# uber/petastorm

Measured on AMD Instinct MI355X. Metric: samples/sec/node (make_batch_reader->PyTorch DataLoader), imagenet config, higher is better.
Workload: dtype fp32; 1 GPU; model=ImageNetSchema(224x224x3 jpeg CompressedImageCodec + int32 label), global_batch=256, parallelism=dp1, prime_batches=0

## Files before the change

petastorm_amd/ops/csrc/ext.cpp:

```cpp
#include <torch/extension.h>

namespace psa {

void snappy_decompress_batch(torch::Tensor comp, torch::Tensor comp_start,
                             torch::Tensor comp_end, torch::Tensor out,
                             torch::Tensor out_offsets,
                             torch::Tensor out_len, torch::Tensor status);
void lz4_decompress_batch(torch::Tensor comp, torch::Tensor blk_start,
                          torch::Tensor blk_end, torch::Tensor out,
                          torch::Tensor out_offsets, torch::Tensor out_len,
                          torch::Tensor status);

void zstd_decompress_host(torch::Tensor src, torch::Tensor src_off,
                          torch::Tensor src_len, torch::Tensor dst,
                          torch::Tensor dst_off, torch::Tensor dst_len,
                          torch::Tensor status);

int64_t zstd_work_bytes();
void zstd_decompress_batch(torch::Tensor src, torch::Tensor src_off,
                           torch::Tensor src_len, torch::Tensor dst,
                           torch::Tensor dst_off, torch::Tensor dst_len,
                           torch::Tensor work, torch::Tensor status);

void rle_hybrid_decode_batch(torch::Tensor data, torch::Tensor start,
                             torch::Tensor end, torch::Tensor bit_width,
                             torch::Tensor n_values, torch::Tensor out_off,
                             torch::Tensor out, torch::Tensor status);
void byte_array_offsets_batch(torch::Tensor data, torch::Tensor start,
                              torch::Tensor end, torch::Tensor n_values,
                              torch::Tensor out_off, torch::Tensor val_off,
                              torch::Tensor val_len, torch::Tensor status);
void varlen_gather(torch::Tensor src, torch::Tensor src_off,
                   torch::Tensor lengths, torch::Tensor dst,
                   torch::Tensor dst_off);
void plain_fixed_decode_batch(torch::Tensor page_buf,
                              torch::Tensor payload_start,
                              torch::Tensor payload_end,
                              torch::Tensor n_values, torch::Tensor row0,
                              int64_t def_mode, int64_t esize,
                              int64_t fill_pattern, torch::Tensor def_buf,
                              torch::Tensor def_start, torch::Tensor def_len,
                              torch::Tensor out,
                              torch::Tensor valid_out, torch::Tensor status);
void npy_payload_offsets(torch::Tensor data, torch::Tensor val_off,
                         torch::Tensor val_len, torch::Tensor pay_off,
                         torch::Tensor pay_len, torch::Tensor status);
void nhwc_to_nchw_normalize(torch::Tensor in, torch::Tensor out,
                            torch::Tensor mean, torch::Tensor inv_std,
                            double scale);
py::dict jpeg_parse_batch(torch::Tensor buf, torch::Tensor val_off,
                          torch::Tensor val_len);
py::dict parquet_walk_pages(torch::Tensor buf, torch::Tensor chunk_off,
                            torch::Tensor chunk_len);
void inflate_batch(torch::Tensor src, torch::Tensor seg_off,
                   torch::Tensor seg_len, torch::Tensor seg_first,
                   torch::Tensor seg_count, torch::Tensor dst,
                   torch::Tensor dst_off, torch::Tensor dst_cap,
                   torch::Tensor produced, int64_t mode,
                   torch::Tensor status);
void png_unfilter_batch(torch::Tensor raw, torch::Tensor raw_off,
                        torch::Tensor out, torch::Tensor out_off,
                        torch::Tensor height, torch::Tensor row_bytes,
                        torch::Tensor bpp, torch::Tensor status);
void bswap16(torch::Tensor data);
py::dict png_parse_batch(torch::Tensor buf, torch::Tensor val_off,
                         torch::Tensor val_len);
py::dict byte_array_host_offsets(torch::Tensor buf, torch::Tensor val_start,
                                 torch::Tensor counts);
void jpeg_decode_batch(torch::Tensor data, py::dict meta, torch::Tensor coef,
                       torch::Tensor samples, torch::Tensor out,
                       torch::Tensor out_off, torch::Tensor status);
void delta_binary_packed_batch(torch::Tensor page_buf, torch::Tensor start,
                               torch::Tensor end, torch::Tensor n_values,
                               torch::Tensor out_off, torch::Tensor out,
                               int64_t esize, torch::Tensor status);
void delta_length_byte_array_batch(torch::Tensor page_buf,
                                   torch::Tensor start, torch::Tensor end,
                                   torch::Tensor n_values,
                                   torch::Tensor out_idx,
                                   torch::Tensor val_off,
                                   torch::Tensor val_len,
                                   torch::Tensor status);
void delta_byte_array_lengths_batch(torch::Tensor page_buf,
                                    torch::Tensor start, torch::Tensor end,
                                    torch::Tensor n_values,
                                    torch::Tensor out_idx,
                                    torch::Tensor pre, torch::Tensor sfx,
                                    torch::Tensor suf_data_pos,
                                    torch::Tensor status);
void delta_byte_array_reconstruct_batch(
    torch::Tensor page_buf, torch::Tensor n_values, torch::Tensor out_idx,
    torch::Tensor pre, torch::Tensor sfx, torch::Tensor suf_data_pos,
    torch::Tensor val_off, torch::Tensor out, torch::Tensor status);
void byte_stream_split_batch(torch::Tensor page_buf, torch::Tensor start,
                             torch::Tensor n_values, torch::Tensor out_off,
                             torch::Tensor out, int64_t esize);
void bool_unpack_batch(torch::Tensor page_buf, torch::Tensor start,
                       torch::Tensor n_values, torch::Tensor out_off,
                       torch::Tensor out);
void jpeg_decode_fused_batch(torch::Tensor data, py::dict meta,
                             torch::Tensor coef, torch::Tensor samples,
                             torch::Tensor out, torch::Tensor out_off,
                             torch::Tensor mean, torch::Tensor inv_std,
                             double scale, torch::Tensor status);

}

PYBIND11_MODULE(TORCH_EXTENSION_NAME, m) {
  m.doc() = "petastorm_amd MI355X (gfx950) decode kernels";
  m.def("snappy_decompress_batch", &psa::snappy_decompress_batch,
        "Batched snappy page decompression (wave-per-page)");
  m.def("lz4_decompress_batch", &psa::lz4_decompress_batch,
        "batch LZ4 block decompression, one wave per block");
  m.def("zstd_decompress_host", &psa::zstd_decompress_host,
        "batch ZSTD frame decompression on host threads (from-scratch "
        "RFC 8878 decoder, GIL released)");
  m.def("zstd_work_bytes", &psa::zstd_work_bytes,
        "per-frame device workspace size for zstd_decompress_batch");
  m.def("zstd_decompress_batch", &psa::zstd_decompress_batch,
        "batch ZSTD frame decompression on device (thread per frame)");
  m.def("rle_hybrid_decode_batch", &psa::rle_hybrid_decode_batch,
        "Parquet RLE/bit-packed hybrid decode (levels & dict indices)");
  m.def("byte_array_offsets_batch", &psa::byte_array_offsets_batch,
        "PLAIN byte-array page -> per-value (offset, length)");
  m.def("varlen_gather", &psa::varlen_gather,
        "Unaligned variable-length byte gather (funnel-shift copy)");
  m.def("plain_fixed_decode_batch", &psa::plain_fixed_decode_batch,
        "Fused PLAIN data-page decode: def levels + prefix scan + scatter");
  m.def("npy_payload_offsets", &psa::npy_payload_offsets,
        ".npy container -> payload (offset, length)");
  m.def("nhwc_to_nchw_normalize", &psa::nhwc_to_nchw_normalize,
        "Fused uint8 NHWC -> float NCHW normalize (LDS-tiled)");
  m.def("parquet_walk_pages", &psa::parquet_walk_pages,
        "Walk Parquet page headers (thrift compact) in a raw column chunk");
  m.def("inflate_batch", &psa::inflate_batch,
        "Batched DEFLATE inflate (zlib/raw), thread-per-stream");
  m.def("png_unfilter_batch", &psa::png_unfilter_batch,
        "PNG scanline unfilter (wave-per-image, bpp-lane chains)");
  m.def("bswap16", &psa::bswap16, "byte-swap 16-bit samples in place");
  m.def("png_parse_batch", &psa::png_parse_batch,
        "Host-side PNG container parse");
  m.def("byte_array_host_offsets", &psa::byte_array_host_offsets,
        "Host-side PLAIN byte-array offset scan");
  m.def("jpeg_parse_batch", &psa::jpeg_parse_batch,
        "Host-side JPEG header/segment parse");
  m.def("jpeg_decode_batch", &psa::jpeg_decode_batch,
        "GPU baseline JPEG decode (huffman/idct/color kernels)");
  m.def("delta_binary_packed_batch", &psa::delta_binary_packed_batch,
        "DELTA_BINARY_PACKED page decode (wave-per-page, shfl prefix scan)");
  m.def("delta_length_byte_array_batch",
        &psa::delta_length_byte_array_batch,
        "DELTA_LENGTH_BYTE_ARRAY page -> per-value (offset, length)");
  m.def("delta_byte_array_lengths_batch",
        &psa::delta_byte_array_lengths_batch,
        "DELTA_BYTE_ARRAY pass 1: prefix/suffix lengths");
  m.def("delta_byte_array_reconstruct_batch",
        &psa::delta_byte_array_reconstruct_batch,
        "DELTA_BYTE_ARRAY pass 2: materialize front-coded values");
  m.def("byte_stream_split_batch", &psa::byte_stream_split_batch,
        "BYTE_STREAM_SPLIT de-interleave");
  m.def("bool_unpack_batch", &psa::bool_unpack_batch,
        "PLAIN boolean bit-unpack");
  m.def("jpeg_decode_fused_batch", &psa::jpeg_decode_fused_batch,
        "JPEG decode with fused YCbCr->RGB + normalize + NCHW fp32 "
        "epilogue (skips the NHWC uint8 intermediate)");
}
```

petastorm_amd/ops/csrc/jpeg.hip:

```cpp
#include <hip/hip_runtime.h>
#include <torch/extension.h>
#include <c10/hip/HIPStream.h>
#include "common.h"

namespace psa {

__constant__ int ZIGZAG_NAT[64] = {
    0,  1,  8,  16, 9,  2,  3,  10, 17, 24, 32, 25, 18, 11, 4,  5,
    12, 19, 26, 33, 40, 48, 41, 34, 27, 20, 13, 6,  7,  14, 21, 28,
    35, 42, 49, 56, 57, 50, 43, 36, 29, 22, 15, 23, 30, 37, 44, 51,
    58, 59, 52, 45, 38, 31, 39, 46, 53, 60, 61, 54, 47, 55, 62, 63};

__constant__ float IDCT_B[8][8] = {
    {0.35355339f, 0.35355339f, 0.35355339f, 0.35355339f,
     0.35355339f, 0.35355339f, 0.35355339f, 0.35355339f},
    {0.49039264f, 0.41573481f, 0.27778512f, 0.09754516f,
     -0.09754516f, -0.27778512f, -0.41573481f, -0.49039264f},
    {0.46193977f, 0.19134172f, -0.19134172f, -0.46193977f,
     -0.46193977f, -0.19134172f, 0.19134172f, 0.46193977f},
    {0.41573481f, -0.09754516f, -0.49039264f, -0.27778512f,
     0.27778512f, 0.49039264f, 0.09754516f, -0.41573481f},
    {0.35355339f, -0.35355339f, -0.35355339f, 0.35355339f,
     0.35355339f, -0.35355339f, -0.35355339f, 0.35355339f},
    {0.27778512f, -0.49039264f, 0.09754516f, 0.41573481f,
     -0.41573481f, -0.09754516f, 0.49039264f, -0.27778512f},
    {0.19134172f, -0.46193977f, 0.46193977f, -0.19134172f,
     -0.19134172f, 0.46193977f, -0.46193977f, 0.19134172f},
    {0.09754516f, -0.27778512f, 0.41573481f, -0.49039264f,
     0.49039264f, -0.41573481f, 0.27778512f, -0.09754516f}};

struct JpegTables {
  const int32_t* lut;
  const int32_t* maxcode;
  const int32_t* mincode;
  const int32_t* valptr;
  const uint8_t* huffval;
  const float* qtabs;
};

struct JpegGeom {
  const int32_t* comp_h;
  const int32_t* comp_v;
  const int32_t* comp_q;
  const int32_t* comp_dc;
  const int32_t* comp_ac;
  const int64_t* samp_off;
  const int32_t* samp_stride;
  const int32_t* mcus_x;
  const int32_t* mcus_y;
  const int32_t* ncomp;
  const int32_t* width;
  const int32_t* height;
  const int64_t* img_block0;
  const int32_t* bpm;
  const int32_t* kmap;
};


struct BitReader {
  const uint8_t* p;
  int64_t pos, end;
  uint64_t buf;
  int cnt;
  uint32_t sw0, sw1;
  int64_t spos;
  int scount;

  __device__ void init(const uint8_t* data, int64_t lo, int64_t hi) {
    p = data; pos = lo; end = hi; buf = 0; cnt = 0; scount = 0; spos = 0;
  }
  __device__ __forceinline__ void fill() {
    while (cnt <= 32) {
      if (pos + 4 <= end) {
        uint32_t w;
        if (scount > 0 && spos == pos) {
          w = sw0;
          sw0 = sw1;
          spos += 4;
          --scount;
        } else {
          scount = 0;
          w = (uint32_t)p[pos] | ((uint32_t)p[pos + 1] << 8) |
              ((uint32_t)p[pos + 2] << 16) | ((uint32_t)p[pos + 3] << 24);
          if (pos + 12 <= end) {
            sw0 = (uint32_t)p[pos + 4] | ((uint32_t)p[pos + 5] << 8) |
// ... 11 lines not shown
            spos = pos + 4;
            scount = 1;
          }
        }
        uint32_t inv = ~w;
        if (!((inv - 0x01010101u) & ~inv & 0x80808080u)) {
          uint32_t be = __builtin_bswap32(w);
          buf |= (uint64_t)be << (32 - cnt);
          cnt += 32;
          pos += 4;
          continue;
        }
      }
      uint8_t b = 0;
      if (pos < end) {
        b = p[pos];
        if (b == 0xFF) {
          if (pos + 1 < end && p[pos + 1] == 0x00) {
            pos += 2;
          } else {
            pos = end;
            b = 0;
          }
        } else {
          pos += 1;
        }
      } else {
        buf |= 0;
        cnt += 8;
        continue;
      }
      buf |= (uint64_t)b << (56 - cnt);
      cnt += 8;
    }
  }
  __device__ __forceinline__ uint32_t peek(int n) {
    return (uint32_t)(buf >> (64 - n));
  }
  __device__ __forceinline__ void consume(int n) {
    buf <<= n;
    cnt -= n;
  }
};

__device__ __forceinline__ int huff_decode(BitReader& br,
                                           const JpegTables& t, int tid) {
  br.fill();
  uint32_t look = br.peek(8);
  int32_t hit = t.lut[tid * 256 + look];
  if (hit >= 0) {
    br.consume(hit >> 16);
    return hit & 0xFF;
  }
  for (int l = 9; l <= 16; ++l) {
    int32_t code = (int32_t)br.peek(l);
    int32_t mc = t.maxcode[tid * 18 + l];
    if (mc >= 0 && code <= mc) {
      br.consume(l);
      int idx = t.valptr[tid * 18 + l] + code - t.mincode[tid * 18 + l];
      return t.huffval[tid * 256 + idx];
    }
  }
  return -1;
}

__device__ __forceinline__ int receive_extend(BitReader& br, int s) {
  br.fill();
  int v = (int)br.peek(s);
  br.consume(s);
  if (v < (1 << (s - 1))) v += (-1 << s) + 1;
  return v;
}

template <bool NT>
__device__ __forceinline__ int decode_block(BitReader& br,
                                            const JpegTables& tabs,
                                            const float* __restrict__ q,
                                            int dc_t, int ac_t,
                                            float* __restrict__ out,
                                            int& pred) {
  int t = huff_decode(br, tabs, dc_t);
  if (t < 0 || t > 15) return 10;
  int diff = t ? receive_extend(br, t) : 0;
  pred += diff;
  if (NT) __builtin_nontemporal_store((float)pred * q[0], out);
  else out[0] = (float)pred * q[0];
  int kk = 1;
  while (kk < 64) {
    int rs = huff_decode(br, tabs, ac_t);
    if (rs < 0) return 11;
    int r = rs >> 4, sz = rs & 15;
    if (sz == 0) {
      if (r != 15) break;
      kk += 16;
    } else {
      kk += r;
      if (kk > 63) return 12;
      int v = receive_extend(br, sz);
      if (NT) __builtin_nontemporal_store((float)v * q[kk],
                                          out + ZIGZAG_NAT[kk]);
      else out[ZIGZAG_NAT[kk]] = (float)v * q[kk];
      ++kk;
    }
  }
  return 0;
}

template <bool NT>
__global__ void jpeg_huffman_kernel(
    const uint8_t* __restrict__ data, JpegTables tabs, JpegGeom g,
    const int32_t* __restrict__ seg_img, const int64_t* __restrict__ seg_pos,
    const int64_t* __restrict__ seg_end, const int32_t* __restrict__ seg_mcu0,
    const int32_t* __restrict__ seg_nmcu, float* __restrict__ coef,
    int32_t* __restrict__ status, int n_segs) {
  int s = blockIdx.x * blockDim.x + threadIdx.x;
  if (s >= n_segs) return;
// ... 42 lines not shown

__global__ void jpeg_idct_kernel(const float* __restrict__ coef,
                                 JpegGeom g, uint8_t* __restrict__ samples,
                                 int n_imgs, int64_t block_total) {
  int64_t b = (int64_t)blockIdx.x * blockDim.x + threadIdx.x;
  if (b >= block_total) return;
  int lo = 0, hi = n_imgs - 1;
  while (lo < hi) {
    int mid = (lo + hi + 1) >> 1;
    if (g.img_block0[mid] <= b) lo = mid; else hi = mid - 1;
  }
  const int img = lo;
  const int bpm = g.bpm[img];
  const int64_t r = b - g.img_block0[img];
  const int m = (int)(r / bpm);
  const int k = (int)(r % bpm);
  const int km = g.kmap[img * 8 + k];
  const int c = km >> 8, v = (km >> 4) & 15, h = km & 15;
  const int mx = m % g.mcus_x[img];
  const int my = m / g.mcus_x[img];
  const int stride = g.samp_stride[img * 3 + c];
  uint8_t* dst = samples + g.samp_off[img * 3 + c] +
                 ((int64_t)(my * g.comp_v[img * 3 + c] + v) * 8) * stride +
                 (int64_t)(mx * g.comp_h[img * 3 + c] + h) * 8;

  const float* C = coef + b * 64;
  float tmp[64];
#pragma unroll
  for (int vv = 0; vv < 8; ++vv) {
#pragma unroll
    for (int x = 0; x < 8; ++x) {
      float acc = 0.f;
#pragma unroll
      for (int u = 0; u < 8; ++u) acc += C[vv * 8 + u] * IDCT_B[u][x];
      tmp[vv * 8 + x] = acc;
    }
  }
#pragma unroll
  for (int y = 0; y < 8; ++y) {
    uint8_t row[8];
#pragma unroll
    for (int x = 0; x < 8; ++x) {
      float acc = 0.f;
#pragma unroll
      for (int vv = 0; vv < 8; ++vv) acc += tmp[vv * 8 + x] * IDCT_B[vv][y];
      int pix = __float2int_rn(acc) + 128;
      row[x] = (uint8_t)min(255, max(0, pix));
    }
    *(uint64_t*)(dst + (int64_t)y * stride) = *(const uint64_t*)row;
  }
}


__device__ __forceinline__ int fancy_sample(const uint8_t* plane, int stride,
                                            int cw, int ch, int x, int y,
                                            int sx, int sy) {
  if (sx == 1 && sy == 1) return plane[(int64_t)y * stride + x] << 4;
  int i = x, j = y, dx = 0, dy = 0;
  if (sx == 2) { i = x >> 1; dx = x & 1; }
  if (sy == 2) { j = y >> 1; dy = y & 1; }
  int i2 = min(max(dx ? i + 1 : i - 1, 0), cw - 1);
  int j2 = min(max(dy ? j + 1 : j - 1, 0), ch - 1);
  if (sx == 2 && sy == 2) {
    int t0 = 3 * plane[(int64_t)j * stride + i] +
             plane[(int64_t)j2 * stride + i];
    int t1 = 3 * plane[(int64_t)j * stride + i2] +
             plane[(int64_t)j2 * stride + i2];
    return (3 * t0 + t1 + (dx ? 7 : 8));
  }
  if (sx == 2) {
    int a = plane[(int64_t)j * stride + i], bq = plane[(int64_t)j * stride + i2];
    return (3 * a + bq + (dx ? 2 : 1)) << 2;
  }
  int a = plane[(int64_t)j * stride + i], bq = plane[(int64_t)j2 * stride + i];
  return (3 * a + bq + (dy ? 2 : 1)) << 2;
}

__global__ void jpeg_color_kernel(const uint8_t* __restrict__ samples,
                                  JpegGeom g,
                                  uint8_t* __restrict__ out,
                                  const int64_t* __restrict__ out_off,
                                  int n_imgs) {
  const int img = blockIdx.y;
  const int W = g.width[img], H = g.height[img];
  const int64_t npix = (int64_t)W * H;
  const int nc = g.ncomp[img];
  const uint8_t* yplane = samples + g.samp_off[img * 3 + 0];
  const int ystride = g.samp_stride[img * 3 + 0];
  uint8_t* dst = out + out_off[img];

  const int hmax = g.comp_h[img * 3 + 0];
  const int vmax = g.comp_v[img * 3 + 0];

  const int Wq = (W + 3) >> 2;
  const int64_t nquads = (int64_t)Wq * H;
  const uint8_t* cbp = samples + g.samp_off[img * 3 + 1];
  const uint8_t* crp = samples + g.samp_off[img * 3 + 2];
  const int cstride = g.samp_stride[img * 3 + 1];
  const int cw = (W + hmax - 1) / hmax;
  const int chh = (H + vmax - 1) / vmax;

  for (int64_t q = (int64_t)blockIdx.x * blockDim.x + threadIdx.x;
       q < nquads; q += (int64_t)gridDim.x * blockDim.x) {
    const int y = (int)(q / Wq);
    const int x0 = (int)(q % Wq) << 2;
    const int cnt = min(4, W - x0);
    const int64_t pix0 = (int64_t)y * W + x0;
    const uint8_t* yrow = yplane + (int64_t)y * ystride + x0;

    if (nc == 1) {
      if (cnt == 4 && (((uintptr_t)(dst + pix0) & 3) == 0) &&
          (((uintptr_t)yrow & 3) == 0))
        *(uint32_t*)(dst + pix0) = *(const uint32_t*)yrow;
      else
        for (int k = 0; k < cnt; ++k) dst[pix0 + k] = yrow[k];
      continue;
    }

    uint8_t rgb[12];
    uint32_t y4 = (cnt == 4) ? load_u32_unaligned(yrow) : 0;
    for (int k = 0; k < cnt; ++k) {
      const int x = x0 + k;
      const float fy = (cnt == 4) ? (float)((y4 >> (8 * k)) & 0xff)
                                  : (float)yrow[k];
      float cb = fancy_sample(cbp, cstride, cw, chh, x, y, hmax, vmax)
                     * (1.f / 16.f) - 128.f;
      float cr = fancy_sample(crp, cstride, cw, chh, x, y, hmax, vmax)
                     * (1.f / 16.f) - 128.f;
      int rv = __float2int_rn(fy + 1.40200f * cr);
      int gv = __float2int_rn(fy - 0.34414f * cb - 0.71414f * cr);
      int bv = __float2int_rn(fy + 1.77200f * cb);
      rgb[k * 3 + 0] = (uint8_t)min(255, max(0, rv));
      rgb[k * 3 + 1] = (uint8_t)min(255, max(0, gv));
      rgb[k * 3 + 2] = (uint8_t)min(255, max(0, bv));
    }
    uint8_t* d = dst + pix0 * 3;
    if (cnt == 4 && (((uintptr_t)d & 3) == 0)) {
      ((uint32_t*)d)[0] = *(const uint32_t*)(rgb + 0);
      ((uint32_t*)d)[1] = *(const uint32_t*)(rgb + 4);
      ((uint32_t*)d)[2] = *(const uint32_t*)(rgb + 8);
    } else {
      for (int k = 0; k < cnt * 3; ++k) d[k] = rgb[k];
    }
  }
}

__global__ void jpeg_color_norm_kernel(
    const uint8_t* __restrict__ samples, JpegGeom g,
    float* __restrict__ out, const int64_t* __restrict__ out_off,
    const float* __restrict__ mean, const float* __restrict__ inv_std,
    float scale, int n_imgs) {
  const int img = blockIdx.y;
  const int W = g.width[img], H = g.height[img];
  const int64_t plane = (int64_t)W * H;
  const int nc = g.ncomp[img];
  const uint8_t* yplane = samples + g.samp_off[img * 3 + 0];
  const int ystride = g.samp_stride[img * 3 + 0];
  float* dst = out + out_off[img];

  const int hmax = g.comp_h[img * 3 + 0];
  const int vmax = g.comp_v[img * 3 + 0];
  const int Wq = (W + 3) >> 2;
  const int64_t nquads = (int64_t)Wq * H;
  const uint8_t* cbp = samples + g.samp_off[img * 3 + 1];
  const uint8_t* crp = samples + g.samp_off[img * 3 + 2];
  const int cstride = g.samp_stride[img * 3 + 1];
  const int cw = (W + hmax - 1) / hmax;
  const int chh = (H + vmax - 1) / vmax;
  const float m0 = mean[0], m1 = mean[1], m2 = mean[2];
  const float s0 = inv_std[0], s1 = inv_std[1], s2 = inv_std[2];

  for (int64_t q = (int64_t)blockIdx.x * blockDim.x + threadIdx.x;
       q < nquads; q += (int64_t)gridDim.x * blockDim.x) {
    const int y = (int)(q / Wq);
    const int x0 = (int)(q % Wq) << 2;
    const int cnt = min(4, W - x0);
    const int64_t pix0 = (int64_t)y * W + x0;
    const uint8_t* yrow = yplane + (int64_t)y * ystride + x0;

    float rpix[4], gpix[4], bpix[4];
    uint32_t y4 = (cnt == 4) ? load_u32_unaligned(yrow) : 0;
    for (int k = 0; k < cnt; ++k) {
      const int x = x0 + k;
      const float fy = (cnt == 4) ? (float)((y4 >> (8 * k)) & 0xff)
                                  : (float)yrow[k];
      int rv, gv, bv;
      if (nc == 1) {
        rv = gv = bv = (int)fy;
      } else {
        float cb = fancy_sample(cbp, cstride, cw, chh, x, y, hmax, vmax)
                       * (1.f / 16.f) - 128.f;
        float cr = fancy_sample(crp, cstride, cw, chh, x, y, hmax, vmax)
                       * (1.f / 16.f) - 128.f;
        rv = __float2int_rn(fy + 1.40200f * cr);
        gv = __float2int_rn(fy - 0.34414f * cb - 0.71414f * cr);
        bv = __float2int_rn(fy + 1.77200f * cb);
      }
      rpix[k] = ((float)min(255, max(0, rv)) * scale - m0) * s0;
      gpix[k] = ((float)min(255, max(0, gv)) * scale - m1) * s1;
      bpix[k] = ((float)min(255, max(0, bv)) * scale - m2) * s2;
    }
    float* dr = dst + pix0;
    float* dg = dst + plane + pix0;
    float* db = dst + 2 * plane + pix0;
    if (cnt == 4 && ((pix0 & 3) == 0)) {
      *(float4*)dr = make_float4(rpix[0], rpix[1], rpix[2], rpix[3]);
      *(float4*)dg = make_float4(gpix[0], gpix[1], gpix[2], gpix[3]);
      *(float4*)db = make_float4(bpix[0], bpix[1], bpix[2], bpix[3]);
    } else {
      for (int k = 0; k < cnt; ++k) {
        dr[k] = rpix[k];
        dg[k] = gpix[k];
        db[k] = bpix[k];
      }
    }
  }
}


static JpegTables make_tables(const py::dict& d) {
  JpegTables t;
  t.lut = d["lut"].cast<torch::Tensor>().data_ptr<int32_t>();
  t.maxcode = d["maxcode"].cast<torch::Tensor>().data_ptr<int32_t>();
  t.mincode = d["mincode"].cast<torch::Tensor>().data_ptr<int32_t>();
  t.valptr = d["valptr"].cast<torch::Tensor>().data_ptr<int32_t>();
  t.huffval = d["huffval"].cast<torch::Tensor>().data_ptr<uint8_t>();
  t.qtabs = d["qtabs"].cast<torch::Tensor>().data_ptr<float>();
  return t;
}

static JpegGeom make_geom(const py::dict& d) {
  JpegGeom g;
  g.comp_h = d["comp_h"].cast<torch::Tensor>().data_ptr<int32_t>();
  g.comp_v = d["comp_v"].cast<torch::Tensor>().data_ptr<int32_t>();
  g.comp_q = d["comp_q"].cast<torch::Tensor>().data_ptr<int32_t>();
  g.comp_dc = d["comp_dc"].cast<torch::Tensor>().data_ptr<int32_t>();
  g.comp_ac = d["comp_ac"].cast<torch::Tensor>().data_ptr<int32_t>();
  g.samp_off = d["samp_off"].cast<torch::Tensor>().data_ptr<int64_t>();
  g.samp_stride = d["samp_stride"].cast<torch::Tensor>().data_ptr<int32_t>();
  g.mcus_x = d["mcus_x"].cast<torch::Tensor>().data_ptr<int32_t>();
  g.mcus_y = d["mcus_y"].cast<torch::Tensor>().data_ptr<int32_t>();
  g.ncomp = d["ncomp"].cast<torch::Tensor>().data_ptr<int32_t>();
  g.width = d["width"].cast<torch::Tensor>().data_ptr<int32_t>();
  g.height = d["height"].cast<torch::Tensor>().data_ptr<int32_t>();
  g.img_block0 = d["img_block0"].cast<torch::Tensor>().data_ptr<int64_t>();
  g.bpm = d["bpm"].cast<torch::Tensor>().data_ptr<int32_t>();
  g.kmap = d["kmap"].cast<torch::Tensor>().data_ptr<int32_t>();
  return g;
}

void jpeg_decode_batch(torch::Tensor data, py::dict meta, torch::Tensor coef,
                       torch::Tensor samples, torch::Tensor out,
                       torch::Tensor out_off, torch::Tensor status) {
  TORCH_CHECK(data.is_cuda() && coef.is_cuda() && samples.is_cuda() &&
              out.is_cuda());
  JpegTables tabs = make_tables(meta);
  JpegGeom g = make_geom(meta);
  auto seg_img = meta["seg_img"].cast<torch::Tensor>();
  auto seg_pos = meta["seg_pos"].cast<torch::Tensor>();
  auto seg_end = meta["seg_end"].cast<torch::Tensor>();
  auto seg_mcu0 = meta["seg_mcu0"].cast<torch::Tensor>();
  auto seg_nmcu = meta["seg_nmcu"].cast<torch::Tensor>();
  int n_segs = (int)seg_img.numel();
  int n_imgs = (int)meta["width"].cast<torch::Tensor>().numel();
  int64_t block_total = coef.numel() / 64;
  hipStream_t stream = c10::hip::getCurrentHIPStream();

  static const bool use_nt = [] {
    const char* e = getenv("PSA_JPEG_NT");
    return e && e[0] == '1';
  }();
  if (use_nt)
    hipLaunchKernelGGL(jpeg_huffman_kernel<true>,
                       dim3((n_segs + 63) / 64), dim3(64), 0, stream,
                       data.data_ptr<uint8_t>(), tabs, g,
                       seg_img.data_ptr<int32_t>(),
                       seg_pos.data_ptr<int64_t>(),
                       seg_end.data_ptr<int64_t>(),
                       seg_mcu0.data_ptr<int32_t>(),
                       seg_nmcu.data_ptr<int32_t>(), coef.data_ptr<float>(),
                       status.data_ptr<int32_t>(), n_segs);
  else
    hipLaunchKernelGGL(jpeg_huffman_kernel<false>,
                       dim3((n_segs + 63) / 64), dim3(64), 0, stream,
                       data.data_ptr<uint8_t>(), tabs, g,
                       seg_img.data_ptr<int32_t>(),
                       seg_pos.data_ptr<int64_t>(),
                       seg_end.data_ptr<int64_t>(),
                       seg_mcu0.data_ptr<int32_t>(),
                       seg_nmcu.data_ptr<int32_t>(), coef.data_ptr<float>(),
                       status.data_ptr<int32_t>(), n_segs);

  hipLaunchKernelGGL(jpeg_idct_kernel,
                     dim3((unsigned)((block_total + 255) / 256)), dim3(256),
                     0, stream, coef.data_ptr<float>(), g,
                     samples.data_ptr<uint8_t>(), n_imgs, block_total);

  int64_t avg_bytes = n_imgs > 0 ? out.numel() / n_imgs : 0;
  int64_t est_blocks = (avg_bytes / 12 + 255) / 256;
  int grid_x = (int)std::min<int64_t>(std::max<int64_t>(est_blocks, 1), 2048);
  hipLaunchKernelGGL(jpeg_color_kernel, dim3(grid_x, n_imgs), dim3(256), 0,
                     stream, samples.data_ptr<uint8_t>(), g,
                     out.data_ptr<uint8_t>(), out_off.data_ptr<int64_t>(),
                     n_imgs);
}

void jpeg_decode_fused_batch(torch::Tensor data, py::dict meta,
                             torch::Tensor coef, torch::Tensor samples,
                             torch::Tensor out, torch::Tensor out_off,
                             torch::Tensor mean, torch::Tensor inv_std,
                             double scale, torch::Tensor status) {
  TORCH_CHECK(data.is_cuda() && coef.is_cuda() && samples.is_cuda() &&
              out.is_cuda() && out.scalar_type() == torch::kFloat32);
  TORCH_CHECK(mean.is_cuda() && inv_std.is_cuda() &&
              mean.numel() == 3 && inv_std.numel() == 3);
  JpegTables tabs = make_tables(meta);
  JpegGeom g = make_geom(meta);
  auto seg_img = meta["seg_img"].cast<torch::Tensor>();
  auto seg_pos = meta["seg_pos"].cast<torch::Tensor>();
  auto seg_end = meta["seg_end"].cast<torch::Tensor>();
  auto seg_mcu0 = meta["seg_mcu0"].cast<torch::Tensor>();
  auto seg_nmcu = meta["seg_nmcu"].cast<torch::Tensor>();
  int n_segs = (int)seg_img.numel();
  int n_imgs = (int)meta["width"].cast<torch::Tensor>().numel();
  int64_t block_total = coef.numel() / 64;
  hipStream_t stream = c10::hip::getCurrentHIPStream();

  static const bool use_nt = [] {
    const char* e = getenv("PSA_JPEG_NT");
    return e && e[0] == '1';
  }();
  if (use_nt)
    hipLaunchKernelGGL(jpeg_huffman_kernel<true>,
                       dim3((n_segs + 63) / 64), dim3(64), 0, stream,
                       data.data_ptr<uint8_t>(), tabs, g,
                       seg_img.data_ptr<int32_t>(),
                       seg_pos.data_ptr<int64_t>(),
                       seg_end.data_ptr<int64_t>(),
                       seg_mcu0.data_ptr<int32_t>(),
                       seg_nmcu.data_ptr<int32_t>(), coef.data_ptr<float>(),
                       status.data_ptr<int32_t>(), n_segs);
  else
    hipLaunchKernelGGL(jpeg_huffman_kernel<false>,
                       dim3((n_segs + 63) / 64), dim3(64), 0, stream,
                       data.data_ptr<uint8_t>(), tabs, g,
                       seg_img.data_ptr<int32_t>(),
                       seg_pos.data_ptr<int64_t>(),
                       seg_end.data_ptr<int64_t>(),
                       seg_mcu0.data_ptr<int32_t>(),
                       seg_nmcu.data_ptr<int32_t>(), coef.data_ptr<float>(),
                       status.data_ptr<int32_t>(), n_segs);

  hipLaunchKernelGGL(jpeg_idct_kernel,
                     dim3((unsigned)((block_total + 255) / 256)), dim3(256),
                     0, stream, coef.data_ptr<float>(), g,
                     samples.data_ptr<uint8_t>(), n_imgs, block_total);

  int64_t avg_px = n_imgs > 0 ? out.numel() / (3 * n_imgs) : 0;
  int64_t est_blocks = (avg_px / 4 + 255) / 256;
  int grid_x = (int)std::min<int64_t>(std::max<int64_t>(est_blocks, 1), 2048);
  hipLaunchKernelGGL(jpeg_color_norm_kernel, dim3(grid_x, n_imgs), dim3(256),
                     0, stream, samples.data_ptr<uint8_t>(), g,
                     out.data_ptr<float>(), out_off.data_ptr<int64_t>(),
                     mean.data_ptr<float>(), inv_std.data_ptr<float>(),
                     (float)scale, n_imgs);
}

}
```

petastorm_amd/ops/csrc/jpeg_host.cpp:

```cpp
#include <torch/extension.h>
#include <cstdint>
#include <cstring>
#include <map>
#include <thread>
#include <vector>

namespace psa {

namespace {

struct HuffTable {
  int32_t lut[256];
  int32_t maxcode[18];
  int32_t mincode[18];
  int32_t valptr[18];
  uint8_t huffval[256];
  bool used = false;
};

struct ImgInfo {
  int w = 0, h = 0, ncomp = 0;
  int comp_h[3] = {1, 1, 1}, comp_v[3] = {1, 1, 1};
  int comp_q[3] = {0, 0, 0};
  int comp_dc[3] = {0, 0, 0}, comp_ac[3] = {0, 0, 0};
  int restart_interval = 0;
  int64_t scan_start = 0, scan_end = 0;
};

bool build_huff(const uint8_t* bits, const uint8_t* vals, int nvals,
                HuffTable& t) {
  uint32_t code = 0;
  int k = 0;
  int codes_of_len[17];
  for (int l = 1; l <= 16; ++l) codes_of_len[l] = bits[l - 1];
  std::memcpy(t.huffval, vals, nvals);
  for (int i = 0; i < 256; ++i) t.lut[i] = -1;
  for (int l = 1; l <= 16; ++l) {
    if (codes_of_len[l]) {
      if (code + (uint32_t)codes_of_len[l] > (1u << l)) return false;
      t.valptr[l] = k;
      t.mincode[l] = code;
      for (int i = 0; i < codes_of_len[l]; ++i) {
        if (l <= 8) {
          int shift = 8 - l;
          int base = code << shift;
          for (int j = 0; j < (1 << shift); ++j)
            t.lut[base + j] = (l << 16) | vals[k];
        }
        ++k;
        ++code;
      }
      t.maxcode[l] = code - 1;
    } else {
      t.maxcode[l] = -1;
      t.mincode[l] = 0;
      t.valptr[l] = 0;
    }
    code <<= 1;
  }
  t.used = true;
  return k == nvals;
}

inline uint16_t be16(const uint8_t* p) {
  return (uint16_t)((p[0] << 8) | p[1]);
}

}

py::dict jpeg_parse_batch(torch::Tensor buf, torch::Tensor val_off,
                          torch::Tensor val_len) {
  TORCH_CHECK(!buf.is_cuda(), "jpeg_parse_batch reads the host copy");
  TORCH_CHECK(buf.scalar_type() == torch::kUInt8);
  const uint8_t* base = buf.data_ptr<uint8_t>();
  const int64_t* off = val_off.data_ptr<int64_t>();
  const int64_t n = val_off.numel();
  const int64_t* vlen64 = nullptr;
  const int32_t* vlen32 = nullptr;
  if (val_len.scalar_type() == torch::kInt64)
    vlen64 = val_len.data_ptr<int64_t>();
  else
    vlen32 = val_len.data_ptr<int32_t>();
  auto vlen = [&](int64_t i) -> int64_t {
    return vlen64 ? vlen64[i] : (int64_t)vlen32[i];
  };

  std::vector<ImgInfo> imgs(n);
  std::vector<std::array<uint16_t, 64>> qpool;
  std::vector<HuffTable> hpool;
  std::map<std::array<uint16_t, 64>, int> qdedup;
  std::map<std::vector<uint8_t>, int> hdedup;

  std::vector<int32_t> seg_img;
  std::vector<int64_t> seg_pos, seg_end;
  std::vector<int32_t> seg_mcu0, seg_nmcu;
  seg_img.reserve(n * 64);
  seg_pos.reserve(n * 64);
  seg_end.reserve(n * 64);
  seg_mcu0.reserve(n * 64);
  seg_nmcu.reserve(n * 64);
// ... 264 lines not shown
  int32_t* CV = comp_v.data_ptr<int32_t>();
  int32_t* CQ = comp_q.data_ptr<int32_t>();
  int32_t* CDC = comp_dc.data_ptr<int32_t>();
  int32_t* CAC = comp_ac.data_ptr<int32_t>();
  int64_t* SOFF = samp_off.data_ptr<int64_t>();
  int32_t* SSTR = samp_stride.data_ptr<int32_t>();
  int64_t* IB0 = img_block0.data_ptr<int64_t>();
  int32_t* BPM = bpm_t.data_ptr<int32_t>();
  int32_t* KMAP = kmap.data_ptr<int32_t>();
  for (int64_t i = 0; i < n; ++i) {
    ImgInfo& im = imgs[i];
    int hmax = 1, vmax = 1;
    for (int c = 0; c < im.ncomp; ++c) {
      hmax = std::max(hmax, im.comp_h[c]);
      vmax = std::max(vmax, im.comp_v[c]);
    }
    int mx = (im.w + 8 * hmax - 1) / (8 * hmax);
    int my = (im.h + 8 * vmax - 1) / (8 * vmax);
    W[i] = im.w;
    H[i] = im.h;
    NC[i] = im.ncomp;
    MX[i] = mx;
    MY[i] = my;
    IB0[i] = block_total;
    int bpm = 0;
    for (int c = 0; c < im.ncomp; ++c) {
      CH[i * 3 + c] = im.comp_h[c];
      CV[i * 3 + c] = im.comp_v[c];
      CQ[i * 3 + c] = im.comp_q[c];
      CDC[i * 3 + c] = im.comp_dc[c];
      CAC[i * 3 + c] = im.comp_ac[c];
      int pw = mx * im.comp_h[c] * 8;
      int ph = my * im.comp_v[c] * 8;
      SOFF[i * 3 + c] = samp_total;
      SSTR[i * 3 + c] = pw;
      samp_total += (int64_t)pw * ph;
      for (int v = 0; v < im.comp_v[c]; ++v)
        for (int hh = 0; hh < im.comp_h[c]; ++hh)
          KMAP[i * 8 + bpm++] = (c << 8) | (v << 4) | hh;
    }
    BPM[i] = bpm;
    block_total += (int64_t)mx * my * bpm;
  }
  IB0[nimg] = block_total;

  int64_t nq = (int64_t)qpool.size();
  torch::Tensor qtabs = torch::empty({std::max<int64_t>(nq, 1), 64}, f32);
  float* QT = qtabs.data_ptr<float>();
  for (int64_t t = 0; t < nq; ++t)
    for (int k2 = 0; k2 < 64; ++k2)
      QT[t * 64 + k2] = (float)qpool[t][k2];

  int64_t nh = (int64_t)hpool.size();
  torch::Tensor lut = torch::empty({std::max<int64_t>(nh, 1), 256}, i32);
  torch::Tensor maxcode = torch::empty({std::max<int64_t>(nh, 1), 18}, i32);
  torch::Tensor mincode = torch::empty({std::max<int64_t>(nh, 1), 18}, i32);
  torch::Tensor valptr = torch::empty({std::max<int64_t>(nh, 1), 18}, i32);
  torch::Tensor huffval = torch::zeros(
      {std::max<int64_t>(nh, 1), 256},
      torch::TensorOptions().dtype(torch::kUInt8));
  for (int64_t t = 0; t < nh; ++t) {
    std::memcpy(lut[t].data_ptr<int32_t>(), hpool[t].lut, 256 * 4);
    std::memcpy(maxcode[t].data_ptr<int32_t>(), hpool[t].maxcode, 18 * 4);
    std::memcpy(mincode[t].data_ptr<int32_t>(), hpool[t].mincode, 18 * 4);
    std::memcpy(valptr[t].data_ptr<int32_t>(), hpool[t].valptr, 18 * 4);
    std::memcpy(huffval[t].data_ptr<uint8_t>(), hpool[t].huffval, 256);
  }

  int64_t ns = (int64_t)seg_img.size();
  torch::Tensor seg_img_t = torch::empty({ns}, i32);
  torch::Tensor seg_pos_t = torch::empty({ns}, i64);
  torch::Tensor seg_end_t = torch::empty({ns}, i64);
  torch::Tensor seg_mcu0_t = torch::empty({ns}, i32);
  torch::Tensor seg_nmcu_t = torch::empty({ns}, i32);
  std::memcpy(seg_img_t.data_ptr<int32_t>(), seg_img.data(), ns * 4);
  std::memcpy(seg_pos_t.data_ptr<int64_t>(), seg_pos.data(), ns * 8);
  std::memcpy(seg_end_t.data_ptr<int64_t>(), seg_end.data(), ns * 8);
  std::memcpy(seg_mcu0_t.data_ptr<int32_t>(), seg_mcu0.data(), ns * 4);
  std::memcpy(seg_nmcu_t.data_ptr<int32_t>(), seg_nmcu.data(), ns * 4);

  py::dict out;
  out["width"] = width;
  out["height"] = height;
  out["ncomp"] = ncomp;
  out["mcus_x"] = mcus_x_t;
  out["mcus_y"] = mcus_y_t;
  out["comp_h"] = comp_h;
  out["comp_v"] = comp_v;
  out["comp_q"] = comp_q;
  out["comp_dc"] = comp_dc;
  out["comp_ac"] = comp_ac;
  out["samp_off"] = samp_off;
  out["samp_stride"] = samp_stride;
  out["samp_total"] = py::int_(samp_total);
  out["img_block0"] = img_block0;
  out["bpm"] = bpm_t;
  out["kmap"] = kmap;
  out["qtabs"] = qtabs;
  out["lut"] = lut;
  out["maxcode"] = maxcode;
  out["mincode"] = mincode;
  out["valptr"] = valptr;
  out["huffval"] = huffval;
  out["seg_img"] = seg_img_t;
  out["seg_pos"] = seg_pos_t;
  out["seg_end"] = seg_end_t;
  out["seg_mcu0"] = seg_mcu0_t;
  out["seg_nmcu"] = seg_nmcu_t;
  out["block_total"] = py::int_(block_total);
  return out;
}

}
```

Baseline: 514,300 samples/sec.

## Add two-level Huffman LUT and tiled 8x2 fast colour-conversion path

Huffman decoding for codes longer than 8 bits now uses a second-level 256-entry subtable instead of a per-length linear search over maxcode, and the host builds these subtables. For 3-component 4:2:0 and 4:4:4 images, the colour kernels now have each thread handle an 8x2 pixel tile. The thread loads luma and chroma with word-wide reads and reuses the chroma taps across the tile, in place of per-pixel fancy_sample gathers. Grid sizing is scaled to the larger per-thread work, and a force_generic_color flag keeps the old path available. The cost is more code and an alignment requirement on samples, plus a correctness risk at image edges.

```diff
diff --git a/petastorm_amd/ops/csrc/ext.cpp b/petastorm_amd/ops/csrc/ext.cpp
--- a/petastorm_amd/ops/csrc/ext.cpp
+++ b/petastorm_amd/ops/csrc/ext.cpp
@@ -69,7 +69,8 @@
                                  torch::Tensor counts);
 void jpeg_decode_batch(torch::Tensor data, py::dict meta, torch::Tensor coef,
                        torch::Tensor samples, torch::Tensor out,
-                       torch::Tensor out_off, torch::Tensor status);
+                       torch::Tensor out_off, torch::Tensor status,
+                       bool force_generic_color);
 void delta_binary_packed_batch(torch::Tensor page_buf, torch::Tensor start,
                                torch::Tensor end, torch::Tensor n_values,
                                torch::Tensor out_off, torch::Tensor out,
@@ -102,7 +103,8 @@
                              torch::Tensor coef, torch::Tensor samples,
                              torch::Tensor out, torch::Tensor out_off,
                              torch::Tensor mean, torch::Tensor inv_std,
-                             double scale, torch::Tensor status);
+                             double scale, torch::Tensor status,
+                             bool force_generic_color);
 
 }
 
@@ -145,7 +147,12 @@
   m.def("jpeg_parse_batch", &psa::jpeg_parse_batch,
         "Host-side JPEG header/segment parse");
   m.def("jpeg_decode_batch", &psa::jpeg_decode_batch,
-        "GPU baseline JPEG decode (huffman/idct/color kernels)");
+        "GPU baseline JPEG decode (huffman/idct/color kernels); "
+        "force_generic_color routes every image through the per-pixel "
+        "colour path (for tests)",
+        py::arg("data"), py::arg("meta"), py::arg("coef"),
+        py::arg("samples"), py::arg("out"), py::arg("out_off"),
+        py::arg("status"), py::arg("force_generic_color") = false);
   m.def("delta_binary_packed_batch", &psa::delta_binary_packed_batch,
         "DELTA_BINARY_PACKED page decode (wave-per-page, shfl prefix scan)");
   m.def("delta_length_byte_array_batch",
@@ -163,5 +170,10 @@
         "PLAIN boolean bit-unpack");
   m.def("jpeg_decode_fused_batch", &psa::jpeg_decode_fused_batch,
         "JPEG decode with fused YCbCr->RGB + normalize + NCHW fp32 "
-        "epilogue (skips the NHWC uint8 intermediate)");
+        "epilogue (skips the NHWC uint8 intermediate); "
+        "force_generic_color as in jpeg_decode_batch",
+        py::arg("data"), py::arg("meta"), py::arg("coef"),
+        py::arg("samples"), py::arg("out"), py::arg("out_off"),
+        py::arg("mean"), py::arg("inv_std"), py::arg("scale"),
+        py::arg("status"), py::arg("force_generic_color") = false);
 }
diff --git a/petastorm_amd/ops/csrc/jpeg.hip b/petastorm_amd/ops/csrc/jpeg.hip
--- a/petastorm_amd/ops/csrc/jpeg.hip
+++ b/petastorm_amd/ops/csrc/jpeg.hip
@@ -31,6 +31,7 @@
 
 struct JpegTables {
   const int32_t* lut;
+  const int32_t* lut2;
   const int32_t* maxcode;
   const int32_t* mincode;
   const int32_t* valptr;
@@ -148,16 +149,10 @@
     br.consume(hit >> 16);
     return hit & 0xFF;
   }
-  for (int l = 9; l <= 16; ++l) {
-    int32_t code = (int32_t)br.peek(l);
-    int32_t mc = t.maxcode[tid * 18 + l];
-    if (mc >= 0 && code <= mc) {
-      br.consume(l);
-      int idx = t.valptr[tid * 18 + l] + code - t.mincode[tid * 18 + l];
-      return t.huffval[tid * 256 + idx];
-    }
-  }
-  return -1;
+  int32_t hit2 = t.lut2[(int64_t)(~hit) * 256 + (br.peek(16) & 0xFF)];
+  if (hit2 < 0) return -1;
+  br.consume(hit2 >> 16);
+  return hit2 & 0xFF;
 }
 
 __device__ __forceinline__ int receive_extend(BitReader& br, int s) {
@@ -306,6 +301,30 @@
 }
 
 
+
+__device__ __forceinline__ int fancy_h2v2_v(int near_row, int far_row) {
+  return 3 * near_row + far_row;
+}
+__device__ __forceinline__ int fancy_h2v2_h(int t0, int t1, int dx) {
+  return (3 * t0 + t1 + (dx ? 7 : 8));
+}
+
+__device__ __forceinline__ void ycc_to_rgb(float fy, int cb16, int cr16,
+                                           int& rv, int& gv, int& bv) {
+  float cb = cb16 * (1.f / 16.f) - 128.f;
+  float cr = cr16 * (1.f / 16.f) - 128.f;
+  rv = __float2int_rn(fy + 1.40200f * cr);
+  gv = __float2int_rn(fy - 0.34414f * cb - 0.71414f * cr);
+  bv = __float2int_rn(fy + 1.77200f * cb);
+}
+
+__device__ __forceinline__ int clamp_u8(int v) { return min(255, max(0, v)); }
+
+__device__ __forceinline__ float norm_px(int v, float scale, float m,
+                                         float s) {
+  return ((float)clamp_u8(v) * scale - m) * s;
+}
+
 __device__ __forceinline__ int fancy_sample(const uint8_t* plane, int stride,
                                             int cw, int ch, int x, int y,
                                             int sx, int sy) {
@@ -316,11 +335,11 @@
   int i2 = min(max(dx ? i + 1 : i - 1, 0), cw - 1);
   int j2 = min(max(dy ? j + 1 : j - 1, 0), ch - 1);
   if (sx == 2 && sy == 2) {
-    int t0 = 3 * plane[(int64_t)j * stride + i] +
-             plane[(int64_t)j2 * stride + i];
-    int t1 = 3 * plane[(int64_t)j * stride + i2] +
-             plane[(int64_t)j2 * stride + i2];
-    return (3 * t0 + t1 + (dx ? 7 : 8));
+    int t0 = fancy_h2v2_v(plane[(int64_t)j * stride + i],
+                          plane[(int64_t)j2 * stride + i]);
+    int t1 = fancy_h2v2_v(plane[(int64_t)j * stride + i2],
+                          plane[(int64_t)j2 * stride + i2]);
+    return fancy_h2v2_h(t0, t1, dx);
   }
   if (sx == 2) {
     int a = plane[(int64_t)j * stride + i], bq = plane[(int64_t)j * stride + i2];
@@ -328,13 +347,113 @@
   }
   int a = plane[(int64_t)j * stride + i], bq = plane[(int64_t)j2 * stride + i];
   return (3 * a + bq + (dy ? 2 : 1)) << 2;
+}
+
+template <bool H2V2, class RowSink>
+__device__ __forceinline__ void color_tile_8x2(
+    const uint8_t* __restrict__ yplane, int ystride,
+    const uint8_t* __restrict__ cbp, const uint8_t* __restrict__ crp,
+    int cstride, int cw, int chh, int x0, int y0, int nrows,
+    RowSink&& sink) {
+  const uint8_t* yr = yplane + (int64_t)y0 * ystride + x0;
+  const uint2 ya = *(const uint2*)yr;
+  const uint2 yb = *(const uint2*)(yr + ystride);
+  const uint32_t yw[2][2] = {{ya.x, ya.y}, {yb.x, yb.y}};
+
+  if (H2V2) {
+    const int i0 = x0 >> 1, j = y0 >> 1;
+    const int jr[3] = {max(j - 1, 0), j, min(j + 1, chh - 1)};
+    const int lim = cw - 1 - i0;
+    const int il = i0 > 0 ? i0 - 4 : i0;
+    const int ir = lim >= 4 ? i0 + 4 : i0;
+    uint32_t cen[2][3], lft[2][3], rgt[2][3];
+#pragma unroll
+    for (int p = 0; p < 2; ++p) {
+#pragma unroll
+      for (int rr = 0; rr < 3; ++rr) {
+        const uint8_t* row = (p ? crp : cbp) + (int64_t)jr[rr] * cstride;
+        cen[p][rr] = *(const uint32_t*)(row + i0);
+        lft[p][rr] = *(const uint32_t*)(row + il);
+        rgt[p][rr] = *(const uint32_t*)(row + ir);
+      }
+    }
+    int tap[2][3][6];
+#pragma unroll
+    for (int p = 0; p < 2; ++p) {
+#pragma unroll
+      for (int rr = 0; rr < 3; ++rr) {
+        const uint32_t c = cen[p][rr];
+        tap[p][rr][1] = (int)(c & 0xff);
+        tap[p][rr][0] = i0 > 0 ? (int)(lft[p][rr] >> 24) : tap[p][rr][1];
+        tap[p][rr][2] = lim >= 1 ? (int)((c >> 8) & 0xff) : tap[p][rr][1];
+        tap[p][rr][3] = lim >= 2 ? (int)((c >> 16) & 0xff) : tap[p][rr][2];
+        tap[p][rr][4] = lim >= 3 ? (int)(c >> 24) : tap[p][rr][3];
+        tap[p][rr][5] = lim >= 4 ? (int)(rgt[p][rr] & 0xff) : tap[p][rr][4];
+      }
+    }
+#pragma unroll
+    for (int r = 0; r < 2; ++r) {
+      if (r < nrows) {
+        int colsum[2][6];
+#pragma unroll
+        for (int p = 0; p < 2; ++p)
+#pragma unroll
+          for (int m = 0; m < 6; ++m)
+            colsum[p][m] = fancy_h2v2_v(tap[p][1][m], tap[p][r ? 2 : 0][m]);
+        int rv[8], gv[8], bv[8];
+#pragma unroll
+        for (int k = 0; k < 8; ++k) {
+          const int a = 1 + (k >> 1), dx = k & 1;
+          const int b = dx ? a + 1 : a - 1;
+          const float fy = (float)((yw[r][k >> 2] >> (8 * (k & 3))) & 0xff);
+          ycc_to_rgb(fy, fancy_h2v2_h(colsum[0][a], colsum[0][b], dx),
+                     fancy_h2v2_h(colsum[1][a], colsum[1][b], dx),
+                     rv[k], gv[k], bv[k]);
+        }
+        sink(r, rv, gv, bv);
+      }
+    }
+  } else {
+    const uint8_t* cbr = cbp + (int64_t)y0 * cstride + x0;
+    const uint8_t* crr = crp + (int64_t)y0 * cstride + x0;
+    const uint2 ba = *(const uint2*)cbr;
+    const uint2 bb = *(const uint2*)(cbr + cstride);
+    const uint2 ra = *(const uint2*)crr;
+    const uint2 rb = *(const uint2*)(crr + cstride);
+    const uint32_t bw[2][2] = {{ba.x, ba.y}, {bb.x, bb.y}};
+    const uint32_t rw[2][2] = {{ra.x, ra.y}, {rb.x, rb.y}};
+#pragma unroll
+    for (int r = 0; r < 2; ++r) {
+      if (r < nrows) {
+        int rv[8], gv[8], bv[8];
+#pragma unroll
+        for (int k = 0; k < 8; ++k) {
+          const int sh = 8 * (k & 3);
+          const float fy = (float)((yw[r][k >> 2] >> sh) & 0xff);
+          ycc_to_rgb(fy, (int)((bw[r][k >> 2] >> sh) & 0xff) << 4,
+                     (int)((rw[r][k >> 2] >> sh) & 0xff) << 4,
+                     rv[k], gv[k], bv[k]);
+        }
+        sink(r, rv, gv, bv);
+      }
+    }
+  }
+}
+
+__device__ __forceinline__ bool color_fast_layout(const JpegGeom& g, int img,
+                                                  int nc, int hmax,
+                                                  int vmax) {
+  return nc == 3 && g.comp_h[img * 3 + 1] == 1 &&
+         g.comp_v[img * 3 + 1] == 1 && g.comp_h[img * 3 + 2] == 1 &&
+         g.comp_v[img * 3 + 2] == 1 &&
+         ((hmax == 2 && vmax == 2) || (hmax == 1 && vmax == 1));
 }
 
 __global__ void jpeg_color_kernel(const uint8_t* __restrict__ samples,
                                   JpegGeom g,
                                   uint8_t* __restrict__ out,
                                   const int64_t* __restrict__ out_off,
-                                  int n_imgs) {
+                                  int n_imgs, bool force_generic) {
   const int img = blockIdx.y;
   const int W = g.width[img], H = g.height[img];
   const int64_t npix = (int64_t)W * H;
@@ -354,6 +473,51 @@
   const int cw = (W + hmax - 1) / hmax;
   const int chh = (H + vmax - 1) / vmax;
 
+  if (!force_generic && color_fast_layout(g, img, nc, hmax, vmax)) {
+    const int Wt = (W + 7) >> 3;
+    const int64_t ntiles = (int64_t)Wt * ((H + 1) >> 1);
+    for (int64_t q = (int64_t)blockIdx.x * blockDim.x + threadIdx.x;
+         q < ntiles; q += (int64_t)gridDim.x * blockDim.x) {
+      const int y0 = (int)(q / Wt) << 1;
+      const int x0 = (int)(q % Wt) << 3;
+      const int cnt = min(8, W - x0);
+      auto sink = [&](int r, const int (&rv)[8], const int (&gv)[8],
+                      const int (&bv)[8]) {
+        uint8_t* d = dst + ((int64_t)(y0 + r) * W + x0) * 3;
+        if (cnt == 8 && (((uintptr_t)d & 3) == 0)) {
+          uint32_t w[6] = {0, 0, 0, 0, 0, 0};
+#pragma unroll
+          for (int k = 0; k < 8; ++k) {
+            w[(3 * k + 0) >> 2] |= (uint32_t)clamp_u8(rv[k])
+                                   << (8 * ((3 * k + 0) & 3));
+            w[(3 * k + 1) >> 2] |= (uint32_t)clamp_u8(gv[k])
+                                   << (8 * ((3 * k + 1) & 3));
+            w[(3 * k + 2) >> 2] |= (uint32_t)clamp_u8(bv[k])
+                                   << (8 * ((3 * k + 2) & 3));
+          }
+#pragma unroll
+          for (int i = 0; i < 6; ++i) ((uint32_t*)d)[i] = w[i];
+        } else {
+#pragma unroll
+          for (int k = 0; k < 8; ++k) {
+            if (k < cnt) {
+              d[3 * k + 0] = (uint8_t)clamp_u8(rv[k]);
+              d[3 * k + 1] = (uint8_t)clamp_u8(gv[k]);
+              d[3 * k + 2] = (uint8_t)clamp_u8(bv[k]);
+            }
+          }
+        }
+      };
+      if (hmax == 2)
+        color_tile_8x2<true>(yplane, ystride, cbp, crp, cstride, cw, chh,
+                             x0, y0, min(2, H - y0), sink);
+      else
+        color_tile_8x2<false>(yplane, ystride, cbp, crp, cstride, cw, chh,
+                              x0, y0, min(2, H - y0), sink);
+    }
+    return;
+  }
+
   for (int64_t q = (int64_t)blockIdx.x * blockDim.x + threadIdx.x;
        q < nquads; q += (int64_t)gridDim.x * blockDim.x) {
     const int y = (int)(q / Wq);
@@ -377,16 +541,13 @@
       const int x = x0 + k;
       const float fy = (cnt == 4) ? (float)((y4 >> (8 * k)) & 0xff)
                                   : (float)yrow[k];
-      float cb = fancy_sample(cbp, cstride, cw, chh, x, y, hmax, vmax)
-                     * (1.f / 16.f) - 128.f;
-      float cr = fancy_sample(crp, cstride, cw, chh, x, y, hmax, vmax)
-                     * (1.f / 16.f) - 128.f;
-      int rv = __float2int_rn(fy + 1.40200f * cr);
-      int gv = __float2int_rn(fy - 0.34414f * cb - 0.71414f * cr);
-      int bv = __float2int_rn(fy + 1.77200f * cb);
-      rgb[k * 3 + 0] = (uint8_t)min(255, max(0, rv));
-      rgb[k * 3 + 1] = (uint8_t)min(255, max(0, gv));
-      rgb[k * 3 + 2] = (uint8_t)min(255, max(0, bv));
+      int rv, gv, bv;
+      ycc_to_rgb(fy, fancy_sample(cbp, cstride, cw, chh, x, y, hmax, vmax),
+                 fancy_sample(crp, cstride, cw, chh, x, y, hmax, vmax),
+                 rv, gv, bv);
+      rgb[k * 3 + 0] = (uint8_t)clamp_u8(rv);
+      rgb[k * 3 + 1] = (uint8_t)clamp_u8(gv);
+      rgb[k * 3 + 2] = (uint8_t)clamp_u8(bv);
     }
     uint8_t* d = dst + pix0 * 3;
     if (cnt == 4 && (((uintptr_t)d & 3) == 0)) {
@@ -403,7 +564,7 @@
     const uint8_t* __restrict__ samples, JpegGeom g,
     float* __restrict__ out, const int64_t* __restrict__ out_off,
     const float* __restrict__ mean, const float* __restrict__ inv_std,
-    float scale, int n_imgs) {
+    float scale, int n_imgs, bool force_generic) {
   const int img = blockIdx.y;
   const int W = g.width[img], H = g.height[img];
   const int64_t plane = (int64_t)W * H;
@@ -424,6 +585,55 @@
   const float m0 = mean[0], m1 = mean[1], m2 = mean[2];
   const float s0 = inv_std[0], s1 = inv_std[1], s2 = inv_std[2];
 
+  if (!force_generic && color_fast_layout(g, img, nc, hmax, vmax)) {
+    const int Wt = (W + 7) >> 3;
+    const int64_t ntiles = (int64_t)Wt * ((H + 1) >> 1);
+    for (int64_t q = (int64_t)blockIdx.x * blockDim.x + threadIdx.x;
+         q < ntiles; q += (int64_t)gridDim.x * blockDim.x) {
+      const int y0 = (int)(q / Wt) << 1;
+      const int x0 = (int)(q % Wt) << 3;
+      const int cnt = min(8, W - x0);
+      auto sink = [&](int r, const int (&rv)[8], const int (&gv)[8],
+                      const int (&bv)[8]) {
+        float* dr = dst + (int64_t)(y0 + r) * W + x0;
+        float* dg = dr + plane;
+        float* db = dg + plane;
+        float rp[8], gp[8], bp[8];
+#pragma unroll
+        for (int k = 0; k < 8; ++k) {
+          rp[k] = norm_px(rv[k], scale, m0, s0);
+          gp[k] = norm_px(gv[k], scale, m1, s1);
+          bp[k] = norm_px(bv[k], scale, m2, s2);
+        }
+        if (cnt == 8 && ((((uintptr_t)dr | (uintptr_t)dg | (uintptr_t)db) &
+                          15) == 0)) {
+          ((float4*)dr)[0] = make_float4(rp[0], rp[1], rp[2], rp[3]);
+          ((float4*)dr)[1] = make_float4(rp[4], rp[5], rp[6], rp[7]);
+          ((float4*)dg)[0] = make_float4(gp[0], gp[1], gp[2], gp[3]);
+          ((float4*)dg)[1] = make_float4(gp[4], gp[5], gp[6], gp[7]);
+          ((float4*)db)[0] = make_float4(bp[0], bp[1], bp[2], bp[3]);
+          ((float4*)db)[1] = make_float4(bp[4], bp[5], bp[6], bp[7]);
+        } else {
+#pragma unroll
+          for (int k = 0; k < 8; ++k) {
+            if (k < cnt) {
+              dr[k] = rp[k];
+              dg[k] = gp[k];
+              db[k] = bp[k];
+            }
+          }
+        }
+      };
+      if (hmax == 2)
+        color_tile_8x2<true>(yplane, ystride, cbp, crp, cstride, cw, chh,
+                             x0, y0, min(2, H - y0), sink);
+      else
+        color_tile_8x2<false>(yplane, ystride, cbp, crp, cstride, cw, chh,
+                              x0, y0, min(2, H - y0), sink);
+    }
+    return;
+  }
+
   for (int64_t q = (int64_t)blockIdx.x * blockDim.x + threadIdx.x;
        q < nquads; q += (int64_t)gridDim.x * blockDim.x) {
     const int y = (int)(q / Wq);
@@ -442,17 +652,14 @@
       if (nc == 1) {
         rv = gv = bv = (int)fy;
       } else {
-        float cb = fancy_sample(cbp, cstride, cw, chh, x, y, hmax, vmax)
-                       * (1.f / 16.f) - 128.f;
-        float cr = fancy_sample(crp, cstride, cw, chh, x, y, hmax, vmax)
-                       * (1.f / 16.f) - 128.f;
-        rv = __float2int_rn(fy + 1.40200f * cr);
-        gv = __float2int_rn(fy - 0.34414f * cb - 0.71414f * cr);
-        bv = __float2int_rn(fy + 1.77200f * cb);
+        ycc_to_rgb(fy,
+                   fancy_sample(cbp, cstride, cw, chh, x, y, hmax, vmax),
+                   fancy_sample(crp, cstride, cw, chh, x, y, hmax, vmax),
+                   rv, gv, bv);
       }
-      rpix[k] = ((float)min(255, max(0, rv)) * scale - m0) * s0;
-      gpix[k] = ((float)min(255, max(0, gv)) * scale - m1) * s1;
-      bpix[k] = ((float)min(255, max(0, bv)) * scale - m2) * s2;
+      rpix[k] = norm_px(rv, scale, m0, s0);
+      gpix[k] = norm_px(gv, scale, m1, s1);
+      bpix[k] = norm_px(bv, scale, m2, s2);
     }
     float* dr = dst + pix0;
     float* dg = dst + plane + pix0;
@@ -475,6 +682,7 @@
 static JpegTables make_tables(const py::dict& d) {
   JpegTables t;
   t.lut = d["lut"].cast<torch::Tensor>().data_ptr<int32_t>();
+  t.lut2 = d["lut2"].cast<torch::Tensor>().data_ptr<int32_t>();
   t.maxcode = d["maxcode"].cast<torch::Tensor>().data_ptr<int32_t>();
   t.mincode = d["mincode"].cast<torch::Tensor>().data_ptr<int32_t>();
   t.valptr = d["valptr"].cast<torch::Tensor>().data_ptr<int32_t>();
@@ -505,9 +713,12 @@
 
 void jpeg_decode_batch(torch::Tensor data, py::dict meta, torch::Tensor coef,
                        torch::Tensor samples, torch::Tensor out,
-                       torch::Tensor out_off, torch::Tensor status) {
+                       torch::Tensor out_off, torch::Tensor status,
+                       bool force_generic_color) {
   TORCH_CHECK(data.is_cuda() && coef.is_cuda() && samples.is_cuda() &&
               out.is_cuda());
+  TORCH_CHECK(((uintptr_t)samples.data_ptr<uint8_t>() & 7) == 0,
+              "samples must be 8-byte aligned");
   JpegTables tabs = make_tables(meta);
   JpegGeom g = make_geom(meta);
   auto seg_img = meta["seg_img"].cast<torch::Tensor>();
@@ -551,21 +762,25 @@
                      samples.data_ptr<uint8_t>(), n_imgs, block_total);
 
   int64_t avg_bytes = n_imgs > 0 ? out.numel() / n_imgs : 0;
-  int64_t est_blocks = (avg_bytes / 12 + 255) / 256;
+  int64_t est_blocks =
+      (avg_bytes / (force_generic_color ? 12 : 48) + 255) / 256;
   int grid_x = (int)std::min<int64_t>(std::max<int64_t>(est_blocks, 1), 2048);
   hipLaunchKernelGGL(jpeg_color_kernel, dim3(grid_x, n_imgs), dim3(256), 0,
                      stream, samples.data_ptr<uint8_t>(), g,
                      out.data_ptr<uint8_t>(), out_off.data_ptr<int64_t>(),
-                     n_imgs);
+                     n_imgs, force_generic_color);
 }
 
 void jpeg_decode_fused_batch(torch::Tensor data, py::dict meta,
                              torch::Tensor coef, torch::Tensor samples,
                              torch::Tensor out, torch::Tensor out_off,
                              torch::Tensor mean, torch::Tensor inv_std,
-                             double scale, torch::Tensor status) {
+                             double scale, torch::Tensor status,
+                             bool force_generic_color) {
   TORCH_CHECK(data.is_cuda() && coef.is_cuda() && samples.is_cuda() &&
               out.is_cuda() && out.scalar_type() == torch::kFloat32);
+  TORCH_CHECK(((uintptr_t)samples.data_ptr<uint8_t>() & 7) == 0,
+              "samples must be 8-byte aligned");
   TORCH_CHECK(mean.is_cuda() && inv_std.is_cuda() &&
               mean.numel() == 3 && inv_std.numel() == 3);
   JpegTables tabs = make_tables(meta);
@@ -611,13 +826,14 @@
                      samples.data_ptr<uint8_t>(), n_imgs, block_total);
 
   int64_t avg_px = n_imgs > 0 ? out.numel() / (3 * n_imgs) : 0;
-  int64_t est_blocks = (avg_px / 4 + 255) / 256;
+  int64_t est_blocks =
+      (avg_px / (force_generic_color ? 4 : 16) + 255) / 256;
   int grid_x = (int)std::min<int64_t>(std::max<int64_t>(est_blocks, 1), 2048);
   hipLaunchKernelGGL(jpeg_color_norm_kernel, dim3(grid_x, n_imgs), dim3(256),
                      0, stream, samples.data_ptr<uint8_t>(), g,
                      out.data_ptr<float>(), out_off.data_ptr<int64_t>(),
                      mean.data_ptr<float>(), inv_std.data_ptr<float>(),
-                     (float)scale, n_imgs);
-}
-
-}
+                     (float)scale, n_imgs, force_generic_color);
+}
+
+}
diff --git a/petastorm_amd/ops/csrc/jpeg_host.cpp b/petastorm_amd/ops/csrc/jpeg_host.cpp
--- a/petastorm_amd/ops/csrc/jpeg_host.cpp
+++ b/petastorm_amd/ops/csrc/jpeg_host.cpp
@@ -1,4 +1,5 @@
 #include <torch/extension.h>
+#include <array>
 #include <cstdint>
 #include <cstring>
 #include <map>
@@ -15,6 +16,7 @@
   int32_t mincode[18];
   int32_t valptr[18];
   uint8_t huffval[256];
+  std::vector<std::array<int32_t, 256>> sub;
   bool used = false;
 };
 
@@ -46,6 +48,20 @@
           int base = code << shift;
           for (int j = 0; j < (1 << shift); ++j)
             t.lut[base + j] = (l << 16) | vals[k];
+        } else {
+          int prefix = (int)(code >> (l - 8));
+          if (t.lut[prefix] == -1) {
+            std::array<int32_t, 256> fresh;
+            fresh.fill(-1);
+            t.sub.push_back(fresh);
+            t.lut[prefix] = ~(int32_t)t.sub.size();
+          }
+          if (t.lut[prefix] >= 0) return false;
+          std::array<int32_t, 256>& st = t.sub[~t.lut[prefix] - 1];
+          int shift = 16 - l;
+          int base = (int)((code << shift) & 0xFF);
+          for (int j = 0; j < (1 << shift); ++j)
+            st[base + j] = (l << 16) | vals[k];
         }
         ++k;
         ++code;
@@ -416,6 +432,9 @@
       QT[t * 64 + k2] = (float)qpool[t][k2];
 
   int64_t nh = (int64_t)hpool.size();
+  int64_t nsub = 1;
+  for (int64_t t = 0; t < nh; ++t) nsub += (int64_t)hpool[t].sub.size();
+  torch::Tensor lut2 = torch::full({nsub, 256}, -1, i32);
   torch::Tensor lut = torch::empty({std::max<int64_t>(nh, 1), 256}, i32);
   torch::Tensor maxcode = torch::empty({std::max<int64_t>(nh, 1), 18}, i32);
   torch::Tensor mincode = torch::empty({std::max<int64_t>(nh, 1), 18}, i32);
@@ -423,8 +442,18 @@
   torch::Tensor huffval = torch::zeros(
       {std::max<int64_t>(nh, 1), 256},
       torch::TensorOptions().dtype(torch::kUInt8));
+  int32_t* L2 = lut2.data_ptr<int32_t>();
+  int64_t sub_base = 1;
   for (int64_t t = 0; t < nh; ++t) {
-    std::memcpy(lut[t].data_ptr<int32_t>(), hpool[t].lut, 256 * 4);
+    int32_t* L1 = lut.data_ptr<int32_t>() + t * 256;
+    for (int k2 = 0; k2 < 256; ++k2) {
+      int32_t e = hpool[t].lut[k2];
+      L1[k2] = e < -1 ? ~(int32_t)(sub_base + (~e - 1)) : e;
+    }
+    for (size_t k2 = 0; k2 < hpool[t].sub.size(); ++k2)
+      std::memcpy(L2 + (sub_base + (int64_t)k2) * 256,
+                  hpool[t].sub[k2].data(), 256 * 4);
+    sub_base += (int64_t)hpool[t].sub.size();
     std::memcpy(maxcode[t].data_ptr<int32_t>(), hpool[t].maxcode, 18 * 4);
     std::memcpy(mincode[t].data_ptr<int32_t>(), hpool[t].mincode, 18 * 4);
     std::memcpy(valptr[t].data_ptr<int32_t>(), hpool[t].valptr, 18 * 4);
@@ -462,6 +491,7 @@
   out["kmap"] = kmap;
   out["qtabs"] = qtabs;
   out["lut"] = lut;
+  out["lut2"] = lut2;
   out["maxcode"] = maxcode;
   out["mincode"] = mincode;
   out["valptr"] = valptr;
```

Result: slower. 495,400 samples/sec (-3.7%).
